# dingwentao/GPU-lossless-compression

Measured on AMD Instinct MI355X. Metric: encode+decode GB/s (input bytes) per GPU and whole-node; compression ratio parity, higher is better.
Workload: dtype u8; 1 GPU; configs[1]: 4 GiB/GPU Zipf(1.0) bytes (Philox4x32-10, key 0x5eed0002, counter = byte index / 4), 1 MiB blocks, cudppCompress BWT+MTF+Huffman encode; block_bytes=1048576, blocks_per_gpu=4096, batch_rows=2048, batch_rows_asked=2048, output_layout=compact, drain_between_steps=False, parallelism=blocks round-robin over 1 GPU(s), no data-path collective, blocks_left_by_bucket_sorter=0, blocks_left_by_sample_sorter=0

## Files before the change

### gpu-lossless-compression_amd/csrc/bwt_bucket.hip

```cpp
#include "glc_device.h"
#include "glc_internal.h"
#include "fs_words.h"

namespace glc {

constexpr int      FSS_NT    = 512;
constexpr int      FSS_ITEMS = FS_CAP / FSS_NT;
#ifndef GLC_FS_BIN_BITS
#define GLC_FS_BIN_BITS 12
#endif
constexpr uint32_t FS_BIN_BITS = GLC_FS_BIN_BITS, FS_BINS = 1u << FS_BIN_BITS;
#ifndef GLC_FSS_LOOK
#define GLC_FSS_LOOK 4
#endif
constexpr uint32_t FSS_LOOK = GLC_FSS_LOOK;
constexpr uint32_t FS_MAX_GROUP = 512;
constexpr uint32_t FS_START_MASK = 0x0FFFu, FS_BIG_BIN = 0x8000u;
static_assert(FS_FILLMAX <= FS_START_MASK, "a bin start and the end of the last bin fit below the big-bin flag");
constexpr uint32_t FSS_SENT = 2 * FSS_LOOK;

uint32_t fs_bucket_log2(uint32_t n)
{
    uint32_t l = 4;
    while (((uint64_t)FS_AVG << l) < n && l < FS_MAXNB_LOG2) l++;
    return l;
}

constexpr uint32_t FSH_SLICE = 32768;
constexpr uint32_t FSH_SLOTS = 2048, FS_DUP_FLAG = 48;

constexpr uint32_t FS_DONE = 8u;

__global__ __launch_bounds__(256) void k_fs_tables(const uint32_t *__restrict__ hist, uint32_t n,
                                                   uint2 *__restrict__ tab, const uint32_t *__restrict__ dup,
                                                   uint32_t *__restrict__ flag, const uint8_t *__restrict__ text, size_t stride,
                                                   uint8_t *__restrict__ bwt_out, size_t bwt_stride, int *__restrict__ d_index,
                                                   uint32_t *__restrict__ sa_out, size_t sa_stride, uint32_t step)
{
    __shared__ uint32_t s_tmp[5];
    const uint32_t b = blockIdx.x, tid = threadIdx.x;
    const uint32_t hraw = hist[(size_t)b * 256 + tid];
    const uint32_t h = hraw + (step > 1 ? 1u : 0u);
    uint32_t ns = 0;
    const uint32_t c = block_excl_add<256>(h, s_tmp, &ns);
    bool constant = __syncthreads_or((int)(hraw == ns - (step > 1 ? 256u : 0u))) != 0;
    if (constant && step > 1) {
        const uint8_t *T = text + (size_t)b * stride;
        const uint32_t sym = T[0];
        bool other = false;
        for (uint32_t i = tid; i < n && !other; i += 256) other = T[i] != sym;
        constant = __syncthreads_or((int)other) == 0;
    }
    if (tid == 0) {
        if (constant) flag[b] = FS_DONE;
        else if (dup[b] >= (FS_DUP_FLAG + step - 1) / step) flag[b] = 1u;
    }
    if (constant) {
        const uint32_t sym = text[(size_t)b * stride];
        const uint32_t v = sym * 0x01010101u;
        if (bwt_out) {
            uint8_t *O = bwt_out + (size_t)b * bwt_stride;
            const uint32_t head = min(n, (uint32_t)((16u - (uint32_t)(reinterpret_cast<uintptr_t>(O) & 15u)) & 15u));
            const uint32_t nvec = (n - head) / 16;
            for (uint32_t i = tid; i < head; i += 256) O[i] = (uint8_t)sym;
            for (uint32_t i = tid; i < nvec; i += 256) reinterpret_cast<uint4 *>(O + head)[i] = make_uint4(v, v, v, v);
            for (uint32_t i = head + nvec * 16 + tid; i < n; i += 256) O[i] = (uint8_t)sym;
        }
        if (sa_out) for (uint32_t i = tid; i < n; i += 256) sa_out[(size_t)b * sa_stride + i] = n - 1 - i;
        if (d_index && tid == 0) d_index[b] = (int)(n - 1);
        return;
    }
    const uint64_t C32 = ((uint64_t)c << 32) / ns, P32 = ((uint64_t)h << 32) / ns;
    tab[(size_t)b * 256 + tid] = make_uint2((uint32_t)(C32 > 0xFFFFFFFFull ? 0xFFFFFFFFull : C32),
                                            (uint32_t)(P32 > 0xFFFFFFFFull ? 0xFFFFFFFFull : P32));
}

#ifndef GLC_FSH_COPIES
#define GLC_FSH_COPIES 16
#endif
constexpr int FSH_COPIES = GLC_FSH_COPIES;
__global__ __launch_bounds__(256) void k_fs_hist(const uint8_t *__restrict__ text, size_t stride, uint32_t n,
                                                 uint32_t *__restrict__ hist, uint32_t *__restrict__ dup, uint32_t step)
{
    __shared__ uint32_t s_h[FSH_COPIES * 257];
    __shared__ uint32_t s_fp[FSH_SLOTS];
    __shared__ uint32_t s_dup;
    const uint32_t b = blockIdx.y, tid = threadIdx.x;
    const uint32_t lo = blockIdx.x * step * FSH_SLICE;
    if (lo >= n) return;
    const uint32_t hi = min(n, lo + FSH_SLICE);
    for (uint32_t i = tid; i < FSH_COPIES * 257; i += 256) s_h[i] = 0;
    for (uint32_t i = tid; i < FSH_SLOTS; i += 256) s_fp[i] = 0;
    if (tid == 0) s_dup = 0;
    __syncthreads();
    const uint8_t *T = text + (size_t)b * stride;
    uint32_t *H = s_h + (tid & (FSH_COPIES - 1)) * 257;
    uint32_t done = lo;
    if ((reinterpret_cast<uintptr_t>(T + lo) & 15) == 0) {
        const uint32_t nvec = (hi - lo) / 16;
        const uint4 *V = reinterpret_cast<const uint4 *>(T + lo);
        uint4 q[8];
#pragma unroll
        for (int r = 0; r < 8; r++) {
            const uint32_t i = r * 256 + tid;
            q[r] = i < nvec ? V[i] : make_uint4(0, 0, 0, 0);
        }
#pragma unroll
        for (int r = 0; r < 8; r += 4) {
            if (r * 256 + tid < nvec) {
                const uint32_t fp = (q[r].x * 0x9E3779B1u + (q[r].y & 0xFFFFu) * 0x85EBCA6Bu) | 1u;
                const uint32_t old = atomicCAS(&s_fp[(fp * 0xC2B2AE35u) >> 21], 0u, fp);
                if (old == fp) atomicAdd(&s_dup, 1u);
            }
        }
#pragma unroll
        for (int r = 0; r < 8; r++) {
            if (r * 256 + tid < nvec) {
                const uint32_t wd[4] = {q[r].x, q[r].y, q[r].z, q[r].w};
#pragma unroll
                for (int k = 0; k < 4; k++) {
                    atomicAdd(&H[wd[k] & 0xFF], 1u);
                    atomicAdd(&H[(wd[k] >> 8) & 0xFF], 1u);
                    atomicAdd(&H[(wd[k] >> 16) & 0xFF], 1u);
                    atomicAdd(&H[wd[k] >> 24], 1u);
                }
            }
        }
        done = lo + nvec * 16;
    }
    for (uint32_t i = done + tid; i < hi; i += 256) atomicAdd(&H[T[i]], 1u);
    __syncthreads();
    uint32_t c = 0;
#pragma unroll
    for (int k = 0; k < FSH_COPIES; k++) c += s_h[k * 257 + tid];
    if (c) atomicAdd(&hist[(size_t)b * 256 + tid], c);
    if (tid == 0 && s_dup) atomicAdd(&dup[b], s_dup);
}

#ifndef GLC_FSP2_T
#define GLC_FSP2_T 4
#endif
constexpr int FSP2_T = GLC_FSP2_T;
#ifndef GLC_FSP2_WAVES
#define GLC_FSP2_WAVES 5
#endif
#ifndef GLC_FSP2_NT
#define GLC_FSP2_NT 512
#endif
#ifndef GLC_FSP2_TILE
#define GLC_FSP2_TILE 4096
#endif
constexpr int FSP2_TILE = GLC_FSP2_TILE;
constexpr int FSP2_NT = GLC_FSP2_NT;

__device__ __forceinline__ void lds_only_barrier()
{
    asm volatile("s_waitcnt lgkmcnt(0)\n\ts_barrier" ::: "memory");
}

template <int NT>
__device__ __forceinline__ uint32_t bucket_excl_add_lds(uint32_t x, uint32_t *s_tmp)
{
    constexpr uint32_t NW = (NT < (int)FS_MAXNB ? NT : FS_MAXNB) / WAVE;
    const uint32_t w = __builtin_amdgcn_readfirstlane(threadIdx.x >> 6);
    const uint32_t inc = wave_incl_add(x);
    if ((threadIdx.x & 63) == 63 && w < NW) s_tmp[w] = inc;
    asm volatile("s_waitcnt lgkmcnt(0)\n\ts_barrier" ::: "memory");
    uint32_t base = 0;
#pragma unroll
    for (uint32_t i = 0; i < NW; i++)
        if (i < w) base += s_tmp[i];
    return base + inc - x;
}

template <int NT, int ITEMS, int WPE>
__global__ __launch_bounds__(NT) __attribute__((amdgpu_waves_per_eu(WPE, 8))) void k_fs_part2(const uint8_t *__restrict__ text, size_t stride, uint32_t n, uint32_t nbl,
                                                     const uint2 *__restrict__ tab, uint64_t *__restrict__ keys, size_t kstride,
                                                     uint32_t *__restrict__ fill, uint32_t *__restrict__ flag,
                                                     uint32_t *__restrict__ zero_bucket, uint32_t tiles_per_wg)
{
    constexpr uint32_t TILE = NT * ITEMS;
    __shared__ struct {
        uint32_t cnt[FS_MAXNB];
        uint16_t start[FS_MAXNB], gbase[FS_MAXNB];
        uint2 tab[256];
        uint32_t tmp[NT / 64 + 1];
        uint32_t flagged;
        uint64_t w[NT * ITEMS];
    } sh;
    uint32_t *s_cnt = sh.cnt, *s_tmp = sh.tmp;
    uint16_t *s_start = sh.start, *s_gbase = sh.gbase;
    uint2 *s_tab = sh.tab;
    uint64_t *s_w = sh.w;
    uint32_t &s_flagged = sh.flagged;
    uint8_t *s_txt = reinterpret_cast<uint8_t *>(s_w);
    uint32_t bx, by;
    xcd_order(bx, by);
    const uint32_t b = by, tid = threadIdx.x;
    const uint32_t ntiles = (n + TILE - 1) / TILE, tile0 = bx * tiles_per_wg;
    if (tile0 >= ntiles) return;
    const uint8_t *T = text + (size_t)b * stride;
    if (tid == 0) s_flagged = flag[b];
    if (tid < 256) s_tab[tid] = tab[(size_t)b * 256 + tid];
    constexpr int NSTG = ((TILE + 16) / 4 + NT - 1) / NT;
    uint32_t stg[NSTG] = {};
    auto inner = [&](uint32_t tile) { const uint32_t base = tile * TILE; return base > 0 && base + TILE + 16 <= n; };
    auto request = [&](uint32_t tile) {
        const uint8_t *D = T + (size_t)tile * TILE - 1;
#pragma unroll
        for (int r = 0; r < NSTG; r++) {
            const uint32_t q = r * NT + tid;
            const uint32_t qq = q < (TILE + 16) / 4 ? q : 0u;
            uint32_t v;
            __builtin_memcpy(&v, D + 4 * (size_t)qq, 4);
            stg[r] = v;
        }
    };
    const uint32_t tend = min(ntiles, tile0 + tiles_per_wg);
    bool have = false;
    if (inner(tile0)) { request(tile0); have = true; }
    uint64_t *K = keys + (size_t)b * kstride;
    static_assert(TILE <= (1u << 20), "a rank inside (tile, bucket) rides in the index field of the word until the scatter");
    constexpr uint32_t LOW = (uint32_t)FS_LOW_MASK;
    auto bucket_of = [&](uint32_t hi) { return __builtin_amdgcn_ubfe(hi, 32u - nbl, nbl); };
    auto tile_body = [&](auto edge_t, uint32_t base, bool next_inner) __attribute__((always_inline)) -> bool {
        constexpr bool EDGE = decltype(edge_t)::value;
        const uint32_t k0 = tid * ITEMS, gi0 = base + k0;
        constexpr int NBY = (ITEMS + FS_DEPTH + 3) / 4;
        uint32_t by4[NBY];
        if (ITEMS % 8 == 0) {
#pragma unroll
            for (int q = 0; q < NBY; q += 2) {
                const uint2 v = *reinterpret_cast<const uint2 *>(s_txt + k0 + 4 * q);
                by4[q] = v.x;
                if (q + 1 < NBY) by4[q + 1] = v.y;
            }
        } else {
#pragma unroll
            for (int q = 0; q < NBY; q++) by4[q] = *reinterpret_cast<const uint32_t *>(s_txt + k0 + 4 * q);
        }
#define FS_BYTE(j) ((by4[(j) >> 2] >> (8 * ((j) & 3))) & 0xFFu)
        uint2 e[ITEMS + FS_DEPTH - 1];
        auto entry = [&](int k) {
            const uint2 t = s_tab[FS_BYTE(1 + k)];
            if constexpr (EDGE) return gi0 + k >= n ? make_uint2(0u, 0u) : t;
            else return t;
        };
#pragma unroll
        for (int k = 0; k < FS_DEPTH - 1; k++) e[k] = entry(k);
        uint32_t xh[ITEMS], xl[ITEMS];
#pragma unroll
        for (int j = 0; j < ITEMS; j++) {
            e[j + FS_DEPTH - 1] = entry(j + FS_DEPTH - 1);
            uint32_t y = e[j + FS_DEPTH - 1].x;
#pragma unroll
            for (int d = FS_DEPTH - 2; d >= 1; d--) y = e[j + d].x + __umulhi(e[j + d].y, y);
            const uint64_t X = ((uint64_t)e[j].x << 32) + (uint64_t)e[j].y * y;
            const uint32_t hi = (uint32_t)(X >> 32), bk = bucket_of(hi);
            uint32_t r = 0;
            if (!EDGE || gi0 + j < n) r = atomicAdd(&s_cnt[bk], 1u);
            xh[j] = hi;
            xl[j] = ((uint32_t)X & ~LOW) | (r << 8);
            if (j == 0 && gi0 == 0) zero_bucket[b] = bk;
        }
        lds_only_barrier();
        uint32_t g = 0, c = 0;
        {
            c = tid < FS_MAXNB ? s_cnt[tid] : 0u;
            const uint32_t start = bucket_excl_add_lds<NT>(c, s_tmp);
            if (c) g = atomicAdd(&fill[(size_t)b * FS_MAXNB + tid], c);
            if (tid < FS_MAXNB) s_start[tid] = (uint16_t)start;
        }
        {
            const uint2 v = *reinterpret_cast<const uint2 *>(s_txt + k0);
            by4[0] = v.x;
            by4[1] = v.y;
#pragma unroll
            for (int j = 0; j < ITEMS; j++) xl[j] |= FS_BYTE(j);
        }
#undef FS_BYTE
        lds_only_barrier();
#pragma unroll
        for (int j = 0; j < ITEMS; j++) {
            asm volatile("" : "+v"(xh[j]), "+v"(xl[j]));
            if (!EDGE || gi0 + j < n) {
                const uint32_t lo = (xl[j] & ~(LOW ^ 0xFFu)) | ((gi0 + j) << 8);
                s_w[s_start[bucket_of(xh[j])] + ((xl[j] >> 8) & 0xFFFFFu)] = ((uint64_t)xh[j] << 32) | lo;
            }
        }
        if (c && g + c > FS_FILLMAX) { atomicOr(&flag[b], 1u); s_flagged = 1; }
        if (tid < FS_MAXNB) s_gbase[tid] = (uint16_t)(g < FS_CAP ? g : FS_CAP);
        if (next_inner) {
#pragma unroll
            for (int r = 0; r < NSTG; r++) asm volatile("" : "+v"(stg[r]));
        }
        lds_only_barrier();
        if constexpr (EDGE) {
            const uint32_t tile_n = min((uint32_t)TILE, n - base);
#pragma unroll
            for (int r = 0; r < ITEMS; r++) {
                const uint32_t p = r * NT + tid;
                if (p < tile_n) {
                    const uint64_t ww = s_w[p];
                    const uint32_t d = bucket_of((uint32_t)(ww >> 32));
                    const uint32_t off = (uint32_t)s_gbase[d] + (p - (uint32_t)s_start[d]);
                    if (off < FS_CAP) K[(size_t)d * FS_CAP + off] = ww;
                }
            }
        } else {
            if (__builtin_amdgcn_readfirstlane(s_flagged)) return false;
#pragma unroll
            for (int r = 0; r < ITEMS; r++) {
                const uint32_t p = r * NT + tid;
                const uint64_t ww = s_w[p];
                const uint32_t d = bucket_of((uint32_t)(ww >> 32));
                K[d * FS_CAP + (uint32_t)s_gbase[d] + (p - (uint32_t)s_start[d])] = ww;
            }
        }
        return true;
    };
#pragma clang loop unroll(disable)
    for (uint32_t tile = tile0; tile < tend; tile++) {
        const uint32_t base = tile * TILE;
        const bool edge = base + TILE + 16 > n;
        if (tid < FS_MAXNB) s_cnt[tid] = 0;
        if (have) {
#pragma unroll
            for (int r = 0; r < NSTG; r++) {
                const uint32_t q = r * NT + tid;
                if (q < (TILE + 16) / 4) reinterpret_cast<uint32_t *>(s_txt)[q] = stg[r];
            }
        } else {
            for (uint32_t k = tid; k < TILE + 16; k += NT) {
                const int64_t g = (int64_t)base - 1 + k;
                s_txt[k] = g < 0 ? T[n - 1] : (g < (int64_t)n ? T[g] : (uint8_t)0);
            }
        }
        lds_only_barrier();
        const bool next_inner = tile + 1 < tend && inner(tile + 1);
        if (next_inner) request(tile + 1);
        if (s_flagged) return;
        const bool go = edge ? tile_body(std::true_type{}, base, next_inner) : tile_body(std::false_type{}, base, next_inner);
        if (!go) return;
        have = next_inner;
        lds_only_barrier();
    }
}

__global__ __launch_bounds__(FS_MAXNB) void k_fs_scan(const uint32_t *__restrict__ fill, uint32_t *__restrict__ fbase,
                                                      uint32_t *__restrict__ flag, const uint32_t *__restrict__ list)
{
    __shared__ uint32_t s_tmp[FS_MAXNB / 64 + 1];
    const uint32_t b = list ? list[blockIdx.x] : blockIdx.x, tid = threadIdx.x;
    const uint32_t f = fill[(size_t)b * FS_MAXNB + tid];
    if (f > FS_FILLMAX) atomicOr(&flag[b], 1u);
    fbase[(size_t)b * FS_MAXNB + tid] = block_excl_add<FS_MAXNB>(f, s_tmp);
}

__global__ __launch_bounds__(FSS_NT) void k_fs_sort(uint32_t n, uint32_t nbl, const uint64_t *__restrict__ keys,
                                                    size_t kstride, const uint32_t *__restrict__ fill,
                                                    const uint32_t *__restrict__ fbase, uint32_t *__restrict__ flag,
                                                    uint8_t *__restrict__ bwt_out, size_t bwt_stride,
                                                    int *__restrict__ d_index, uint32_t *__restrict__ sa_out,
                                                    size_t sa_stride, uint4 *__restrict__ wl, uint32_t wl_cap,
                                                    uint32_t *__restrict__ wl_count)
{
    __shared__ uint64_t s_w[FS_FILLMAX + 4];
    __shared__ uint32_t s_cp[FS_BINS / 2 + 1];
    __shared__ uint32_t s_tmp[FSS_NT / 64 + 1];
    __shared__ uint32_t s_deep, s_wl;
    uint16_t *s16 = reinterpret_cast<uint16_t *>(s_cp);
    uint8_t *s_cb = reinterpret_cast<uint8_t *>(s_cp);
    uint32_t gx, gy;
    xcd_order(gx, gy);
    const uint32_t b = gy, bk = gx, tid = threadIdx.x;
    if (tid == 0) { s_deep = flag[b]; s_wl = 0; }
    for (uint32_t i = tid; i < FS_BINS / 2; i += FSS_NT) s_cp[i] = 0;
    const uint32_t c = fill[(size_t)b * FS_MAXNB + bk];
    const uint32_t R0 = fbase[(size_t)b * FS_MAXNB + bk];
    const uint64_t *K = keys + (size_t)b * kstride + (size_t)bk * FS_CAP;
    uint64_t w[FSS_ITEMS];
#pragma unroll
    for (int r = 0; r < FSS_ITEMS; r++) {
        const uint32_t i = r * FSS_NT + tid;
        w[r] = ~0ull;
        if (r * FSS_NT < c && c <= FS_FILLMAX && i < c) w[r] = K[i];
    }
    if (tid < 4 && c <= FS_FILLMAX) s_w[c + tid] = ~0ull;
    __syncthreads();
    if (s_deep || c == 0) return;
    const uint32_t bshift = 64 - nbl - FS_BIN_BITS;
    uint32_t rk[FSS_ITEMS];
#pragma unroll
    for (int r = 0; r < FSS_ITEMS; r++) {
        rk[r] = 0;
        if (r * FSS_NT >= c) continue;
        const uint32_t i = r * FSS_NT + tid;
        const uint32_t bin = (uint32_t)(w[r] >> bshift) & (FS_BINS - 1), sh = 16 * (bin & 1);
        if (i < c) rk[r] = (atomicAdd(&s_cp[bin >> 1], 1u << sh) >> sh) & 0xFFFFu;
    }
    __syncthreads();
    {
        constexpr int PW = FS_BINS / 2 / FSS_NT;
        uint32_t v[PW], sum = 0;
#pragma unroll
        for (int k = 0; k < PW; k++) { v[k] = s_cp[tid * PW + k]; sum += (v[k] & 0xFFFFu) + (v[k] >> 16); }
        uint32_t run = block_excl_add<FSS_NT>(sum, s_tmp);
#pragma unroll
        for (int k = 0; k < PW; k++) {
            const uint32_t lo = run, hi = run + (v[k] & 0xFFFFu);
            s_cp[tid * PW + k] = lo | (hi << 16);
            run = hi + (v[k] >> 16);
        }
        if (tid == FSS_NT - 1) s_cp[FS_BINS / 2] = c;
    }
    __syncthreads();
#pragma unroll
    for (int r = 0; r < FSS_ITEMS; r++) {
        if (r * FSS_NT >= c) continue;
        const uint32_t i = r * FSS_NT + tid;
        if (i < c) s_w[s16[(uint32_t)(w[r] >> bshift) & (FS_BINS - 1)] + rk[r]] = w[r];
    }
    __syncthreads();
    uint32_t *SAo = sa_out ? sa_out + (size_t)b * sa_stride + R0 : nullptr;
    uint32_t pos[FSS_ITEMS], grp[FSS_ITEMS];
#pragma unroll
    for (int r = 0; r < FSS_ITEMS; r++) {
        const uint32_t p = r * FSS_NT + tid;
        pos[r] = 0xFFFFFFFFu; grp[r] = 0;
        if (r * FSS_NT >= c) continue;
        if (p < c) {
            const uint64_t wv = s_w[p];
            w[r] = wv;
            const uint32_t key = (uint32_t)(wv >> 28);
            const uint32_t bin = (uint32_t)(wv >> bshift) & (FS_BINS - 1);
            const uint32_t gs = s16[bin], ge = s16[bin + 1];
            if (ge - gs > FS_MAX_GROUP) { s_deep = 1; }
            else {
                uint32_t less = 0, eqt = 0;
                const uint2 *B = reinterpret_cast<const uint2 *>(s_w) + gs;
#pragma unroll
                for (uint32_t t = 0; t < 4; t++) {
                    const uint2 wq = B[t];
                    const uint32_t kq = __builtin_amdgcn_alignbit(wq.y, wq.x, 28);
                    less += kq < key ? 1u : 0u;
                    eqt += kq == key ? 1u : 0u;
                }
                if (ge - gs > 4) {
#pragma clang loop unroll(disable)
                    for (uint32_t q = gs + 4; q < ge; q++) {
                        const uint2 wq = reinterpret_cast<const uint2 *>(s_w)[q];
                        const uint32_t kq = __builtin_amdgcn_alignbit(wq.y, wq.x, 28);
                        less += kq < key; eqt += kq == key;
                    }
                }
                const uint32_t idx = (uint32_t)(wv >> 8) & 0xFFFFFu;
                uint32_t at = gs + less;
                if (eqt > 1) {
                    uint32_t eqb = 0; eqt = 0;
#pragma clang loop unroll(disable)
                    for (uint32_t q = gs; q < ge; q++) {
                        const uint2 wq = reinterpret_cast<const uint2 *>(s_w)[q];
                        const bool e = __builtin_amdgcn_alignbit(wq.y, wq.x, 28) == key;
                        eqt += e; eqb += e & (q < p);
                    }
                    if (eqt > 1) { grp[r] = (at << 16) | eqt; at += eqb; }
                }
                pos[r] = at;
                if (!grp[r]) {
                    if (SAo) SAo[at] = idx;
                    if (idx == 0 && d_index) d_index[b] = (int)(R0 + at);
                }
            }
        }
    }
    __syncthreads();
    if (s_deep) { if (tid == 0) atomicOr(&flag[b], 2u); return; }
    uint8_t *O = bwt_out ? bwt_out + (size_t)b * bwt_stride + R0 : nullptr;
    const uint32_t shift = (uint32_t)(reinterpret_cast<uintptr_t>(O) & 3u);
    bool any = false;
#pragma unroll
    for (int r = 0; r < FSS_ITEMS; r++) {
        if (pos[r] != 0xFFFFFFFFu) s_cb[shift + pos[r]] = (uint8_t)w[r];
        if (grp[r]) {
            any = true;
            const uint32_t gp = grp[r] >> 16, gs = grp[r] & 0xFFFFu;
            if (pos[r] == gp) reinterpret_cast<uint32_t *>(s_w)[2 * gp + 1] = atomicAdd(&s_wl, gs);
        }
    }
    if (__syncthreads_or((int)any)) {
        if (tid == 0) {
            const uint32_t tot = s_wl;
            uint32_t base = atomicAdd(&wl_count[b], tot);
            if (base + tot > wl_cap) { atomicOr(&flag[b], 4u); base = 0xFFFFFFFFu; }
            s_deep = base;
        }
        __syncthreads();
        const uint32_t base = s_deep;
        uint4 *WL = wl + (size_t)b * wl_cap;
        if (base != 0xFFFFFFFFu) {
#pragma unroll
            for (int r = 0; r < FSS_ITEMS; r++) {
                if (grp[r]) {
                    const uint32_t gp = grp[r] >> 16, gs = grp[r] & 0xFFFFu, slot0 = base + reinterpret_cast<const uint32_t *>(s_w)[2 * gp + 1];
                    WL[slot0 + (pos[r] - gp)] = make_uint4((uint32_t)(w[r] & FS_LOW_MASK), R0 + gp, slot0, gs);
                }
            }
        }
    }
    if (O) {
        const uint32_t end = shift + c;
        for (uint32_t q = tid; 4 * q < end; q += FSS_NT) {
            const uint32_t v = s_cp[q];
            if (4 * q >= shift && 4 * q + 4 <= end) *reinterpret_cast<uint32_t *>(O - shift + 4 * q) = v;
            else {
#pragma unroll
                for (uint32_t k = 0; k < 4; k++)
                    if (4 * q + k >= shift && 4 * q + k < end) O[4 * q + k - shift] = (uint8_t)(v >> (8 * k));
            }
        }
    }
}

__global__ __launch_bounds__(FSS_NT) __attribute__((amdgpu_waves_per_eu(8, 8))) void k_fs_sort_bwt(uint32_t nbl, const uint64_t *__restrict__ keys, size_t kstride,
                                                        const uint32_t *__restrict__ fill, const uint32_t *__restrict__ fbase,
                                                        uint32_t *__restrict__ flag, uint8_t *__restrict__ bwt_out,
                                                        size_t bwt_stride, int *__restrict__ d_index, uint4 *__restrict__ wl,
                                                        uint32_t wl_cap, uint32_t *__restrict__ wl_count,
                                                        const uint32_t *__restrict__ zero_bucket)
{
    __shared__ uint64_t s_w[FS_FILLMAX + FSS_SENT];
    __shared__ uint32_t s_cp[FS_BINS / 2 + 1];
    __shared__ uint32_t s_tmp[FSS_NT / 64 + 1];
    __shared__ uint32_t s_deep, s_wl;
    uint16_t *s16 = reinterpret_cast<uint16_t *>(s_cp);
    uint8_t *s_cb = reinterpret_cast<uint8_t *>(s_cp);
    uint32_t gx, gy;
    xcd_order(gx, gy);
    const uint32_t b = gy, bk = gx, tid = threadIdx.x;
    if (scalar_load_u32(flag + b) & (1u | FS_DONE)) return;
    if (tid == 0) { s_deep = flag[b]; s_wl = 0; }
    for (uint32_t i = tid; i < FS_BINS / 2; i += FSS_NT) s_cp[i] = 0;
    const uint64_t *K = keys + (size_t)b * kstride + (size_t)bk * FS_CAP;
    constexpr int FSS_SPEC = 3;
    uint64_t ws[FSS_SPEC + 1];
#pragma unroll
    for (int r = 1; r <= FSS_SPEC; r++) ws[r] = K[(r - 1) * FSS_NT + tid];
    const uint32_t c = fill[(size_t)b * FS_MAXNB + bk];
    const uint32_t R0 = fbase[(size_t)b * FS_MAXNB + bk];
    const bool zb = zero_bucket[b] == bk;
    const uint32_t cc = c <= FS_FILLMAX ? c : 0u;
    const uint32_t full = cc / FSS_NT, part = cc % FSS_NT;
    const bool v0 = tid < part;
    const uint32_t i0 = full * FSS_NT + tid;
    const uint32_t bshift = 64 - nbl - FS_BIN_BITS;
    const uint32_t hshift = bshift - 32, kshift = bshift - 28;
    uint8_t *O = bwt_out + (size_t)b * bwt_stride + R0;
    const uint32_t shift = (uint32_t)(reinterpret_cast<uintptr_t>(O) & 3u);

    auto bin_starts = [&]() __attribute__((always_inline)) {
        constexpr int PW = FS_BINS / 2 / FSS_NT;
        uint32_t v[PW], sum = 0;
#pragma unroll
        for (int k = 0; k < PW; k++) { v[k] = s_cp[tid * PW + k]; sum += (v[k] & 0xFFFFu) + (v[k] >> 16); }
        uint32_t run = block_excl_add<FSS_NT>(sum, s_tmp);
#pragma unroll
        for (int k = 0; k < PW; k++) {
            const uint32_t lo = run, hi = run + (v[k] & 0xFFFFu);
            s_cp[tid * PW + k] = lo | (hi << 16);
            run = hi + (v[k] >> 16);
        }
        if (tid == FSS_NT - 1) s_cp[FS_BINS / 2] = c;
    };
    auto sorted_word = [](uint64_t wv) -> uint64_t {
        const uint32_t lo = (uint32_t)wv, hi = (uint32_t)(wv >> 32);
        return ((uint64_t)__builtin_amdgcn_alignbit(hi, lo, 28) << 32) | lo;
    };
    auto rank_rare = [&](uint32_t key, uint32_t p, uint32_t gs, uint32_t ge, uint32_t &at, uint32_t &grp) __attribute__((always_inline)) {
        if (ge - gs > FS_MAX_GROUP) { s_deep = 1; at = 0xFFFFFFFFu; }
        else {
            uint32_t ls = 0, eq = 0, eqb = 0;
#pragma clang loop unroll(disable)
            for (uint32_t q = gs; q < ge; q++) {
                const uint32_t kq = reinterpret_cast<const uint32_t *>(s_w)[2 * q + 1];
                ls += kq < key; eq += kq == key; eqb += (kq == key) & (q < p);
            }
            at = gs + ls;
            if (eq > 1) { grp = (at << 16) | eq; at += eqb; }
        }
    };
    auto rank_rare2 = [&](uint32_t key, uint32_t p, uint32_t gs, const uint32_t *k1, uint32_t &at, uint32_t &grp) __attribute__((always_inline)) {
        const uint32_t *B = reinterpret_cast<const uint32_t *>(s_w) + 2 * (gs + FSS_LOOK) + 1;
        uint32_t k2[FSS_LOOK];
#pragma unroll
        for (uint32_t t = 0; t < FSS_LOOK; t++) k2[t] = B[2 * t];
        const uint32_t ge = s16[((key >> kshift) & (FS_BINS - 1)) + 1] & FS_START_MASK;
        if ((ge - gs > 2 * FSS_LOOK) | (key == 0xFFFFFFFFu)) rank_rare(key, p, gs, ge, at, grp);
        else {
            uint32_t ls = 0, em = 0;
#pragma unroll
            for (uint32_t t = 0; t < 2 * FSS_LOOK; t++) {
                const uint32_t kq = t < FSS_LOOK ? k1[t < FSS_LOOK ? t : 0] : k2[t < FSS_LOOK ? 0 : t - FSS_LOOK];
                ls += kq < key ? 1u : 0u;
                em |= kq == key ? 1u << t : 0u;
            }
            const uint32_t eq = __builtin_popcount(em);
            at = gs + ls;
            if (eq > 1) { grp = (at << 16) | eq; at += __builtin_popcount(em & ((1u << (p - gs)) - 1u)); }
        }
    };
    auto wl_reserve = [&](uint32_t pos, uint32_t grp) __attribute__((always_inline)) {
        const uint32_t gp = grp >> 16, gs = grp & 0xFFFFu;
        if (pos == gp) reinterpret_cast<uint32_t *>(s_w)[2 * gp + 1] = atomicAdd(&s_wl, gs);
    };
    auto wl_base = [&]() __attribute__((always_inline)) -> uint32_t {
        __syncthreads();
        const uint32_t tot = s_wl;
        if (tot == 0) return 0xFFFFFFFFu;
        if (tid == 0) {
            uint32_t base = atomicAdd(&wl_count[b], tot);
            if (base + tot > wl_cap) { atomicOr(&flag[b], 4u); base = 0xFFFFFFFFu; }
            s_deep = base;
        }
        __syncthreads();
        return s_deep;
    };
    auto wl_entry = [&](uint32_t base, uint64_t wv, uint32_t pos, uint32_t grp) __attribute__((always_inline)) {
        uint4 *WL = wl + (size_t)b * wl_cap;
        const uint32_t gp = grp >> 16, gs = grp & 0xFFFFu, slot0 = base + reinterpret_cast<const uint32_t *>(s_w)[2 * gp + 1];
        WL[slot0 + (pos - gp)] = make_uint4((uint32_t)(wv & FS_LOW_MASK), R0 + gp, slot0, gs);
    };

    auto rounds = [&](auto full_t) __attribute__((always_inline)) -> bool {
        constexpr int FULL = decltype(full_t)::value, NS = FULL + 1;
        static_assert(FULL >= FSS_SPEC && NS <= FSS_ITEMS, "the requested rounds are all full ones");
        uint64_t w[NS];
        w[0] = ~0ull;
        if (v0) w[0] = K[i0];
#pragma unroll
        for (int r = 1; r <= FULL; r++) w[r] = r <= FSS_SPEC ? ws[r <= FSS_SPEC ? r : 0] : K[(r - 1) * FSS_NT + tid];
        if (tid < FSS_SENT) s_w[cc + tid] = ~0ull;
        __syncthreads();
        if (s_deep) return false;
        uint32_t bin[NS], rk[NS];
#pragma unroll
        for (int r = 0; r < NS; r++) bin[r] = ((uint32_t)(w[r] >> 32) >> hshift) & (FS_BINS - 1);
        rk[0] = 0;
        if (v0) rk[0] = atomicAdd(&s_cp[bin[0] >> 1], 1u << (16 * (bin[0] & 1)));
#pragma unroll
        for (int r = 1; r < NS; r++) rk[r] = atomicAdd(&s_cp[bin[r] >> 1], 1u << (16 * (bin[r] & 1)));
#pragma unroll
        for (int r = 0; r < NS; r++) rk[r] = (rk[r] >> (16 * (bin[r] & 1))) & 0xFFFFu;
        __syncthreads();
        bin_starts();
        __syncthreads();
        {
            uint32_t st[NS];
            st[0] = 0;
            if (v0) st[0] = s16[bin[0]];
#pragma unroll
            for (int r = 1; r < NS; r++) st[r] = s16[bin[r]];
            bool late = false;
#pragma unroll
            for (int r = 0; r < NS; r++) late |= rk[r] >= FSS_LOOK;
            if (late) {
#pragma unroll
                for (int r = 0; r < NS; r++)
                    if (rk[r] >= FSS_LOOK) atomicOr(&s_cp[bin[r] >> 1], FS_BIG_BIN << (16 * (bin[r] & 1)));
            }
#pragma unroll
            for (int r = 0; r < NS; r++) rk[r] += st[r] & FS_START_MASK;
            if (v0) s_w[rk[0]] = sorted_word(w[0]);
        }
#pragma unroll
        for (int r = 1; r < NS; r++) s_w[rk[r]] = sorted_word(w[r]);
        __syncthreads();
        uint32_t pos[NS], grp[NS], gs[NS];
        bool big[NS];
        if (v0) w[0] = s_w[i0];
#pragma unroll
        for (int r = 1; r < NS; r++) w[r] = s_w[(r - 1) * FSS_NT + tid];
        gs[0] = 0;
        if (v0) gs[0] = s16[((uint32_t)(w[0] >> 32) >> kshift) & (FS_BINS - 1)];
#pragma unroll
        for (int r = 1; r < NS; r++) gs[r] = s16[((uint32_t)(w[r] >> 32) >> kshift) & (FS_BINS - 1)];
#pragma unroll
        for (int r = 0; r < NS; r++) { big[r] = gs[r] > FS_START_MASK; gs[r] &= FS_START_MASK; }
        uint32_t kq[NS][FSS_LOOK];
        if (v0) {
            const uint32_t *B = reinterpret_cast<const uint32_t *>(s_w) + 2 * gs[0] + 1;
#pragma unroll
            for (uint32_t t = 0; t < FSS_LOOK; t++) kq[0][t] = B[2 * t];
        }
#pragma unroll
        for (int r = 1; r < NS; r++) {
            const uint32_t *B = reinterpret_cast<const uint32_t *>(s_w) + 2 * gs[r] + 1;
#pragma unroll
            for (uint32_t t = 0; t < FSS_LOOK; t++) kq[r][t] = B[2 * t];
        }
        bool rare[NS], rare_any = false;
#pragma unroll
        for (int r = 0; r < NS; r++) {
            const uint32_t key = (uint32_t)(w[r] >> 32);
            uint32_t less = 0, eqt = 0;
#pragma unroll
            for (uint32_t t = 0; t < FSS_LOOK; t++) {
                less += kq[r][t] < key ? 1u : 0u;
                eqt += kq[r][t] == key ? 1u : 0u;
            }
            pos[r] = gs[r] + less; grp[r] = 0;
            rare[r] = (big[r] | (eqt > 1)) & (r > 0 || v0);
            rare_any |= rare[r];
        }
        if (__builtin_amdgcn_ballot_w64(rare_any) != 0) {
#pragma unroll
            for (int r = 0; r < NS; r++)
                if (rare[r]) rank_rare2((uint32_t)(w[r] >> 32), r ? (r - 1) * FSS_NT + tid : i0, gs[r], kq[r], pos[r], grp[r]);
        }
        if (zb) {
            asm volatile("" ::: "memory");
#pragma unroll
            for (int r = 0; r < NS; r++)
                if ((r > 0 || v0) && pos[r] != 0xFFFFFFFFu && ((uint32_t)w[r] & 0x0FFFFF00u) == 0 && !grp[r]) d_index[b] = (int)(R0 + pos[r]);
        }
        __syncthreads();
        if (s_deep) { if (tid == 0) atomicOr(&flag[b], 2u); return false; }
        if (v0) s_cb[shift + pos[0]] = (uint8_t)w[0];
#pragma unroll
        for (int r = 1; r < NS; r++) s_cb[shift + pos[r]] = (uint8_t)w[r];
        uint32_t tied = 0;
#pragma unroll
        for (int r = 0; r < NS; r++) tied |= grp[r];
        if (tied) {
#pragma unroll
            for (int r = 0; r < NS; r++)
                if (grp[r]) wl_reserve(pos[r], grp[r]);
        }
        const uint32_t base = wl_base();
        if (base != 0xFFFFFFFFu && tied) {
#pragma unroll
            for (int r = 0; r < NS; r++)
                if (grp[r]) wl_entry(base, w[r], pos[r], grp[r]);
        }
        return true;
    };

    auto guarded = [&]() __attribute__((always_inline)) -> bool {
        uint64_t w[FSS_ITEMS];
#pragma unroll
        for (int r = 0; r < FSS_ITEMS; r++) w[r] = r >= 1 && r <= FSS_SPEC ? ws[r >= 1 && r <= FSS_SPEC ? r : 0] : ~0ull;
        if (v0) w[0] = K[i0];
#pragma unroll
        for (int r = FSS_SPEC + 1; r < FSS_ITEMS; r++)
            if ((uint32_t)r <= full) w[r] = K[(r - 1) * FSS_NT + tid];
        if (tid < FSS_SENT && cc) s_w[cc + tid] = ~0ull;
        __syncthreads();
        if (s_deep || cc == 0) return false;
        uint32_t rk[FSS_ITEMS];
#pragma unroll
        for (int r = 0; r < FSS_ITEMS; r++) rk[r] = 0;
        {
            auto count = [&](int r) {
                const uint32_t bin = ((uint32_t)(w[r] >> 32) >> hshift) & (FS_BINS - 1), sh = 16 * (bin & 1);
                rk[r] = (atomicAdd(&s_cp[bin >> 1], 1u << sh) >> sh) & 0xFFFFu;
            };
            if (v0) count(0);
#pragma unroll
            for (int r = 1; r < FSS_ITEMS; r++)
                if ((uint32_t)r <= full) count(r);
        }
        __syncthreads();
        bin_starts();
        __syncthreads();
        {
            auto scatter = [&](int r) {
                const uint32_t bin = ((uint32_t)(w[r] >> 32) >> hshift) & (FS_BINS - 1);
                const uint32_t st = s16[bin];
                if (rk[r] >= FSS_LOOK) atomicOr(&s_cp[bin >> 1], FS_BIG_BIN << (16 * (bin & 1)));
                s_w[(st & FS_START_MASK) + rk[r]] = sorted_word(w[r]);
            };
            if (v0) scatter(0);
#pragma unroll
            for (int r = 1; r < FSS_ITEMS; r++)
                if ((uint32_t)r <= full) scatter(r);
        }
        __syncthreads();
        uint32_t pos[FSS_ITEMS], grp[FSS_ITEMS];
#pragma unroll
        for (int r = 0; r < FSS_ITEMS; r++) { pos[r] = 0xFFFFFFFFu; grp[r] = 0; }
        {
            auto rank = [&](int r, uint32_t p) {
                const uint64_t wv = s_w[p];
                w[r] = wv;
                const uint32_t key = (uint32_t)(wv >> 32);
                const uint32_t bin = (key >> kshift) & (FS_BINS - 1);
                const uint32_t gf = s16[bin], gs = gf & FS_START_MASK;
                uint32_t less = 0, eqt = 0, kq[FSS_LOOK];
                const uint32_t *B = reinterpret_cast<const uint32_t *>(s_w) + 2 * gs + 1;
#pragma unroll
                for (uint32_t t = 0; t < FSS_LOOK; t++) {
                    kq[t] = B[2 * t];
                    less += kq[t] < key ? 1u : 0u;
                    eqt += kq[t] == key ? 1u : 0u;
                }
                uint32_t at = gs + less;
                const bool rare = (gf > FS_START_MASK) | (eqt > 1);
                if (__builtin_amdgcn_ballot_w64(rare) != 0) {
                    if (rare) rank_rare2(key, p, gs, kq, at, grp[r]);
                }
                pos[r] = at;
            };
            if (v0) rank(0, i0);
#pragma unroll
            for (int r = 1; r < FSS_ITEMS; r++)
                if ((uint32_t)r <= full) rank(r, (r - 1) * FSS_NT + tid);
            if (zb) {
                asm volatile("" ::: "memory");
#pragma unroll
                for (int r = 0; r < FSS_ITEMS; r++)
                    if (pos[r] != 0xFFFFFFFFu && ((uint32_t)w[r] & 0x0FFFFF00u) == 0 && !grp[r]) d_index[b] = (int)(R0 + pos[r]);
            }
        }
        __syncthreads();
        if (s_deep) { if (tid == 0) atomicOr(&flag[b], 2u); return false; }
#pragma unroll
        for (int r = 0; r < FSS_ITEMS; r++) {
            if (pos[r] != 0xFFFFFFFFu) s_cb[shift + pos[r]] = (uint8_t)w[r];
            if (grp[r]) wl_reserve(pos[r], grp[r]);
        }
        const uint32_t base = wl_base();
        if (base != 0xFFFFFFFFu) {
#pragma unroll
            for (int r = 0; r < FSS_ITEMS; r++)
                if (grp[r]) wl_entry(base, w[r], pos[r], grp[r]);
        }
        return true;
    };

    const bool go = full == 3 ? rounds(std::integral_constant<int, 3>{}) : full == 4 ? rounds(std::integral_constant<int, 4>{}) : guarded();
    if (!go) return;
    {
        const uint32_t end = shift + c;
        for (uint32_t q = tid; 4 * q < end; q += FSS_NT) {
            const uint32_t v = s_cp[q];
            if (4 * q >= shift && 4 * q + 4 <= end) *reinterpret_cast<uint32_t *>(O - shift + 4 * q) = v;
            else {
#pragma unroll
                for (uint32_t k = 0; k < 4; k++)
                    if (4 * q + k >= shift && 4 * q + k < end) O[4 * q + k - shift] = (uint8_t)(v >> (8 * k));
            }
        }
    }
}

#ifndef GLC_FST_W
#define GLC_FST_W 4
#endif
constexpr int FST_W = GLC_FST_W;
__global__ __launch_bounds__(256) void k_fs_ties(const uint8_t *__restrict__ text, size_t stride, uint32_t n,
                                                 const uint4 *__restrict__ wl, uint32_t wl_cap,
                                                 const uint32_t *__restrict__ wl_count, uint32_t *__restrict__ flag,
                                                 uint8_t *__restrict__ bwt_out, size_t bwt_stride,
                                                 int *__restrict__ d_index, uint32_t *__restrict__ sa_out, size_t sa_stride)
{
    uint32_t gx, gy;
    xcd_order(gx, gy);
    const uint32_t b = gy;
    const uint32_t total = wl_count[b];
    if (total == 0 || total > wl_cap || flag[b]) return;
    const uint4 *WL = wl + (size_t)b * wl_cap;
    const uint8_t *T = text + (size_t)b * stride;
    for (uint32_t e = gx * 256 + threadIdx.x; e < total; e += gridDim.x * 256) {
        const uint4 me = WL[e];
        const uint32_t gs = me.w, idx = me.x >> 8;
        uint32_t rank = 0;
        bool deep = false;
        const bool fast_me = idx + 12 <= n;
        const uint64_t mine = fast_me ? fs_load_be64(T + idx) : 0ull;
        for (uint32_t f0 = me.z; f0 < me.z + gs && !deep; f0 += FST_W) {
            uint32_t oi[FST_W];
            uint64_t ov[FST_W];
#pragma unroll
            for (int k = 0; k < FST_W; k++) oi[k] = f0 + k < me.z + gs ? WL[f0 + k].x >> 8 : idx;
#pragma unroll
            for (int k = 0; k < FST_W; k++) ov[k] = (oi[k] != idx && fast_me && oi[k] + 12 <= n) ? fs_load_be64(T + oi[k]) : mine;
#pragma unroll
            for (int k = 0; k < FST_W; k++) {
                if (oi[k] == idx) continue;
                if (fast_me && oi[k] + 12 <= n && ov[k] != mine) rank += ov[k] < mine ? 1u : 0u;
                else rank += fs_suffix_less(T, n, oi[k], idx, &deep) ? 1u : 0u;
            }
        }
        if (deep) { atomicOr(&flag[b], 2u); continue; }
        const uint32_t row = me.y + rank;
        if (bwt_out) bwt_out[(size_t)b * bwt_stride + row] = (uint8_t)me.x;
        if (sa_out) sa_out[(size_t)b * sa_stride + row] = idx;
        if (idx == 0 && d_index) d_index[b] = (int)row;
    }
}

__global__ void k_fs_finish(const uint32_t *__restrict__ flag, uint32_t n, uint32_t nblk, uint32_t *__restrict__ lcnt,
                            uint32_t *__restrict__ nflag, uint32_t *__restrict__ redo, uint32_t *__restrict__ keep,
                            uint32_t *__restrict__ list, uint32_t *__restrict__ h_nflag, const uint32_t *__restrict__ dup,
                            uint32_t dup_flag)
{
    __shared__ uint32_t s_last;
    const uint32_t b = blockIdx.x * blockDim.x + threadIdx.x;
    if (b < nblk) {
        const uint32_t f = (flag[b] && flag[b] != FS_DONE) ? n : 0u;
        lcnt[b] = f;
        redo[b] = f;
        keep[b] = f ? 0u : 1u;
        if (f) list[atomicAdd(nflag, 1u)] = b;
        if (flag[b] != FS_DONE && dup[b] < dup_flag) atomicAdd(nflag + 4, 1u);
    }
    __threadfence();
    __syncthreads();
    if (threadIdx.x == 0) s_last = atomicAdd(&nflag[3], 1u) == gridDim.x - 1 ? 1u : 0u;
    __syncthreads();
    if (s_last && threadIdx.x == 0) {
        __threadfence();
        reinterpret_cast<volatile uint32_t *>(h_nflag)[1] = atomicAdd(nflag + 4, 0u);
        *reinterpret_cast<volatile uint32_t *>(h_nflag) = atomicAdd(nflag, 0u);
        __threadfence_system();
    }
}

__global__ __launch_bounds__(256) void k_fs_clear(uint32_t nblk, uint32_t *__restrict__ hist, uint32_t *__restrict__ fill,
                                                  uint32_t *__restrict__ flag, uint32_t flag_value, uint32_t *__restrict__ wlcnt,
                                                  uint32_t *__restrict__ dup, uint32_t *__restrict__ nflag)
{
    const uint32_t nh = nblk * 256u, nf = nblk * FS_MAXNB, total = nh + nf + 3u * nblk + 8u;
    for (uint32_t i = blockIdx.x * 256u + threadIdx.x; i < total; i += gridDim.x * 256u) {
        if (i < nh) hist[i] = 0;
        else if (i < nh + nf) fill[i - nh] = 0;
        else {
            const uint32_t j = i - nh - nf;
            if (j < nblk) flag[j] = flag_value;
            else if (j < 2 * nblk) wlcnt[j - nblk] = 0;
            else if (j < 3 * nblk) dup[j - 2 * nblk] = 0;
            else nflag[j - 3 * nblk] = 0;
        }
    }
}

hipError_t fs_scan(hipStream_t st, uint32_t nlisted, const uint32_t *fill, uint32_t *fbase, uint32_t *flag, const uint32_t *list)
{
    hipLaunchKernelGGL(k_fs_scan, dim3(nlisted), dim3(FS_MAXNB), 0, st, fill, fbase, flag, list);
    return hipGetLastError();
}

hipError_t fs_build(const SortCall &c, SaScratch &s)
{
    const hipStream_t st = c.st;
    const uint8_t *const text = c.text;
    const size_t text_stride = c.text_stride, bwt_stride = c.bwt_stride;
    const uint32_t n = c.n, nblk = c.nblk;
    uint8_t *const bwt_out = c.bwt_out;
    int *const d_index = c.d_index;
    uint32_t *const sa_out = c.sa_out(s);
    const uint32_t nbl = fs_bucket_log2(n), nb = 1u << nbl;
    {
        const uint32_t words = nblk * (256u + FS_MAXNB + 3u) + 8u, g = (words + 1023) / 1024;
        hipLaunchKernelGGL(k_fs_clear, dim3(g < 2048 ? g : 2048), dim3(256), 0, st, nblk, s.fs_hist, s.fs_fill, s.fs_flag,
                           s.skip_tier1 ? 1u : 0u, s.fs_wlcnt, s.fs_dup, s.fs_nflag);
    }
    uint32_t *h_nflag = s.h_max_cnt + HW_FLAGGED;
    const double units = (double)n * nblk;
    const uint32_t nslices = (n + FSH_SLICE - 1) / FSH_SLICE;
    const uint32_t hstep = nslices >= 16 ? 4u : 1u;
    {
        ProfScope ps(s.prof, PROF_FS_HIST, st, units);
        hipLaunchKernelGGL(k_fs_hist, dim3((nslices + hstep - 1) / hstep, nblk), dim3(256), 0, st, text, text_stride, n,
                           s.fs_hist, s.fs_dup, hstep);
    }
    hipLaunchKernelGGL(k_fs_tables, dim3(nblk), dim3(256), 0, st, s.fs_hist, n, s.fs_tab, s.fs_dup, s.fs_flag, text, text_stride,
                       bwt_out, bwt_stride, d_index, sa_out, (size_t)s.nmax, hstep);
    if (s.skip_tier1) {
        hipLaunchKernelGGL(k_fs_finish, dim3((nblk + 255) / 256), dim3(256), 0, st, s.fs_flag, n, nblk, s.fs_lcnt, s.fs_nflag,
                           s.fs_redo[s.parity & 1], s.fs_keep[s.parity & 1], s.ss_list, h_nflag, s.fs_dup, (FS_DUP_FLAG + hstep - 1) / hstep);
        return hipGetLastError();
    }
    {
        ProfScope ps(s.prof, PROF_FS_PART, st, units);
        if (nblk >= 16) {
#ifndef GLC_FSP2_BT
#define GLC_FSP2_BT 8192
#endif
            constexpr int BT = GLC_FSP2_BT, BN = 1024;
            const uint32_t tiles = (n + BT - 1) / BT, per = 16;
            hipLaunchKernelGGL((k_fs_part2<BN, BT / BN, 4>), dim3((tiles + per - 1) / per, nblk), dim3(BN), 0, st, text, text_stride, n, nbl,
                               s.fs_tab, s.keyA, s.fs_kstride, s.fs_fill, s.fs_flag, s.fs_zero, per);
        } else {
            const uint32_t tiles = (n + FSP2_TILE - 1) / FSP2_TILE;
            const uint32_t per = nblk >= 4 ? FSP2_T : 1u;
            hipLaunchKernelGGL((k_fs_part2<FSP2_NT, FSP2_TILE / FSP2_NT, GLC_FSP2_WAVES>), dim3((tiles + per - 1) / per, nblk), dim3(FSP2_NT), 0, st,
                               text, text_stride, n, nbl, s.fs_tab, s.keyA, s.fs_kstride, s.fs_fill, s.fs_flag, s.fs_zero, per);
        }
    }
    hipLaunchKernelGGL(k_fs_scan, dim3(nblk), dim3(FS_MAXNB), 0, st, s.fs_fill, s.fs_base, s.fs_flag, (const uint32_t *)nullptr);
    {
        ProfScope ps(s.prof, PROF_FS_SORT, st, units);
        if (sa_out || !bwt_out || !d_index)
            hipLaunchKernelGGL(k_fs_sort, dim3(nb, nblk), dim3(FSS_NT), 0, st, n, nbl, s.keyA, s.fs_kstride, s.fs_fill, s.fs_base, s.fs_flag,
                               bwt_out, bwt_stride, d_index, sa_out, (size_t)s.nmax, s.fs_wl, s.fs_wl_cap, s.fs_wlcnt);
        else
            hipLaunchKernelGGL(k_fs_sort_bwt, dim3(nb, nblk), dim3(FSS_NT), 0, st, nbl, s.keyA, s.fs_kstride, s.fs_fill, s.fs_base, s.fs_flag,
                               bwt_out, bwt_stride, d_index, s.fs_wl, s.fs_wl_cap, s.fs_wlcnt, s.fs_zero);
    }
    hipLaunchKernelGGL(k_fs_ties, dim3(24, nblk), dim3(256), 0, st, text, text_stride, n, s.fs_wl, s.fs_wl_cap, s.fs_wlcnt,
                       s.fs_flag, bwt_out, bwt_stride, d_index, sa_out, (size_t)s.nmax);
    hipLaunchKernelGGL(k_fs_finish, dim3((nblk + 255) / 256), dim3(256), 0, st, s.fs_flag, n, nblk, s.fs_lcnt, s.fs_nflag,
                       s.fs_redo[s.parity & 1], s.fs_keep[s.parity & 1], s.ss_list, h_nflag, s.fs_dup, (FS_DUP_FLAG + hstep - 1) / hstep);
    return hipGetLastError();
}

}
```

Before: 122.7 GB/s.

## Feed inner tiles' text bytes straight from registers, skipping LDS staging

For interior tiles, each thread now loads its own 16 bytes of text with one vector load into registers and uses them directly for the code computation. This replaces staging the tile into LDS and reading it back, which also removes a barrier per tile. The loop is restructured so edge tiles keep the LDS path while runs of interior tiles prefetch the next tile's registers. s_cnt is cleared inside the body instead of at the top of each tile. It relies on ITEMS==8 and FS_DEPTH==8 (static_assert), and the reworked barrier ordering between edge and inner tiles adds correctness risk.

```diff
diff --git a/gpu-lossless-compression_amd/csrc/bwt_bucket.hip b/gpu-lossless-compression_amd/csrc/bwt_bucket.hip
--- a/gpu-lossless-compression_amd/csrc/bwt_bucket.hip
+++ b/gpu-lossless-compression_amd/csrc/bwt_bucket.hip
@@ -202,42 +202,36 @@
     const uint8_t *T = text + (size_t)b * stride;
     if (tid == 0) s_flagged = flag[b];
     if (tid < 256) s_tab[tid] = tab[(size_t)b * 256 + tid];
-    constexpr int NSTG = ((TILE + 16) / 4 + NT - 1) / NT;
-    uint32_t stg[NSTG] = {};
+    if (tid < FS_MAXNB) s_cnt[tid] = 0;
+    static_assert(ITEMS == 8 && FS_DEPTH == 8, "a thread's codes and BWT bytes come from the 16 bytes of one load");
+    constexpr int NBY = (ITEMS + FS_DEPTH + 3) / 4;
+    uint32_t nxt[NBY] = {};
     auto inner = [&](uint32_t tile) { const uint32_t base = tile * TILE; return base > 0 && base + TILE + 16 <= n; };
     auto request = [&](uint32_t tile) {
-        const uint8_t *D = T + (size_t)tile * TILE - 1;
-#pragma unroll
-        for (int r = 0; r < NSTG; r++) {
-            const uint32_t q = r * NT + tid;
-            const uint32_t qq = q < (TILE + 16) / 4 ? q : 0u;
-            uint32_t v;
-            __builtin_memcpy(&v, D + 4 * (size_t)qq, 4);
-            stg[r] = v;
-        }
+        uint4 v;
+        __builtin_memcpy(&v, T + (size_t)tile * TILE - 1 + ITEMS * tid, 16);
+        nxt[0] = v.x; nxt[1] = v.y; nxt[2] = v.z; nxt[3] = v.w;
     };
     const uint32_t tend = min(ntiles, tile0 + tiles_per_wg);
-    bool have = false;
-    if (inner(tile0)) { request(tile0); have = true; }
+    if (inner(tile0)) request(tile0);
     uint64_t *K = keys + (size_t)b * kstride;
     static_assert(TILE <= (1u << 20), "a rank inside (tile, bucket) rides in the index field of the word until the scatter");
     constexpr uint32_t LOW = (uint32_t)FS_LOW_MASK;
     auto bucket_of = [&](uint32_t hi) { return __builtin_amdgcn_ubfe(hi, 32u - nbl, nbl); };
-    auto tile_body = [&](auto edge_t, uint32_t base, bool next_inner) __attribute__((always_inline)) -> bool {
+    auto tile_body = [&](auto edge_t, uint32_t base, const uint32_t (&txt)[NBY]) __attribute__((always_inline)) -> bool {
         constexpr bool EDGE = decltype(edge_t)::value;
         const uint32_t k0 = tid * ITEMS, gi0 = base + k0;
-        constexpr int NBY = (ITEMS + FS_DEPTH + 3) / 4;
         uint32_t by4[NBY];
-        if (ITEMS % 8 == 0) {
-#pragma unroll
-            for (int q = 0; q < NBY; q += 2) {
+#pragma unroll
+        for (int q = 0; q < NBY; q += 2) {
+            if constexpr (EDGE) {
                 const uint2 v = *reinterpret_cast<const uint2 *>(s_txt + k0 + 4 * q);
                 by4[q] = v.x;
-                if (q + 1 < NBY) by4[q + 1] = v.y;
-            }
-        } else {
-#pragma unroll
-            for (int q = 0; q < NBY; q++) by4[q] = *reinterpret_cast<const uint32_t *>(s_txt + k0 + 4 * q);
+                by4[q + 1] = v.y;
+            } else {
+                by4[q] = txt[q];
+                by4[q + 1] = txt[q + 1];
+            }
         }
 #define FS_BYTE(j) ((by4[(j) >> 2] >> (8 * ((j) & 3))) & 0xFFu)
         uint2 e[ITEMS + FS_DEPTH - 1];
@@ -267,14 +261,17 @@
         uint32_t g = 0, c = 0;
         {
             c = tid < FS_MAXNB ? s_cnt[tid] : 0u;
+            if (tid < FS_MAXNB) s_cnt[tid] = 0;
             const uint32_t start = bucket_excl_add_lds<NT>(c, s_tmp);
             if (c) g = atomicAdd(&fill[(size_t)b * FS_MAXNB + tid], c);
             if (tid < FS_MAXNB) s_start[tid] = (uint16_t)start;
         }
         {
-            const uint2 v = *reinterpret_cast<const uint2 *>(s_txt + k0);
-            by4[0] = v.x;
-            by4[1] = v.y;
+            if constexpr (EDGE) {
+                const uint2 v = *reinterpret_cast<const uint2 *>(s_txt + k0);
+                by4[0] = v.x;
+                by4[1] = v.y;
+            }
 #pragma unroll
             for (int j = 0; j < ITEMS; j++) xl[j] |= FS_BYTE(j);
         }
@@ -290,10 +287,8 @@
         }
         if (c && g + c > FS_FILLMAX) { atomicOr(&flag[b], 1u); s_flagged = 1; }
         if (tid < FS_MAXNB) s_gbase[tid] = (uint16_t)(g < FS_CAP ? g : FS_CAP);
-        if (next_inner) {
-#pragma unroll
-            for (int r = 0; r < NSTG; r++) asm volatile("" : "+v"(stg[r]));
-        }
+#pragma unroll
+        for (int r = 0; r < NBY; r++) asm volatile("" : "+v"(nxt[r]));
         lds_only_barrier();
         if constexpr (EDGE) {
             const uint32_t tile_n = min((uint32_t)TILE, n - base);
@@ -319,31 +314,38 @@
         }
         return true;
     };
+    lds_only_barrier();
+#pragma unroll
+    for (int r = 0; r < NBY; r++) asm volatile("" : "+v"(nxt[r]));
+    uint32_t tile = tile0;
 #pragma clang loop unroll(disable)
-    for (uint32_t tile = tile0; tile < tend; tile++) {
-        const uint32_t base = tile * TILE;
-        const bool edge = base + TILE + 16 > n;
-        if (tid < FS_MAXNB) s_cnt[tid] = 0;
-        if (have) {
-#pragma unroll
-            for (int r = 0; r < NSTG; r++) {
-                const uint32_t q = r * NT + tid;
-                if (q < (TILE + 16) / 4) reinterpret_cast<uint32_t *>(s_txt)[q] = stg[r];
-            }
-        } else {
+    while (tile < tend) {
+        if (__builtin_amdgcn_readfirstlane(s_flagged)) return;
+        if (!inner(tile)) {
+            const uint32_t base = tile * TILE;
+            if (tile != tile0) lds_only_barrier();
             for (uint32_t k = tid; k < TILE + 16; k += NT) {
                 const int64_t g = (int64_t)base - 1 + k;
                 s_txt[k] = g < 0 ? T[n - 1] : (g < (int64_t)n ? T[g] : (uint8_t)0);
             }
-        }
-        lds_only_barrier();
-        const bool next_inner = tile + 1 < tend && inner(tile + 1);
-        if (next_inner) request(tile + 1);
-        if (s_flagged) return;
-        const bool go = edge ? tile_body(std::true_type{}, base, next_inner) : tile_body(std::false_type{}, base, next_inner);
-        if (!go) return;
-        have = next_inner;
-        lds_only_barrier();
+            lds_only_barrier();
+            if (tile + 1 < tend && inner(tile + 1)) request(tile + 1);
+            tile_body(std::true_type{}, base, nxt);
+            tile++;
+            continue;
+        }
+        bool next_inner;
+#pragma clang loop unroll(disable)
+        do {
+            uint32_t txt[NBY];
+#pragma unroll
+            for (int q = 0; q < NBY; q++) txt[q] = nxt[q];
+            next_inner = tile + 1 < tend && inner(tile + 1);
+            if (next_inner) request(tile + 1);
+            if (!tile_body(std::false_type{}, tile * TILE, txt)) return;
+            lds_only_barrier();
+            tile++;
+        } while (next_inner);
     }
 }
 
```

Result: no change. 121.9 GB/s (-0.6%).

## Split inner-tile key build into load/compute/atomic phases and separate edge loop

Applied to the files above, without the earlier changes.

For interior tiles the bucket-scatter kernel now loads every lookup-table entry first, then computes all codes and LDS atomics, then reads the bucket starts before the scatter stores. Scheduling barriers mark the phase boundaries so LDS loads can be batched and their latency overlapped. The tile loop is restructured so edge tiles take a separate path and interior tiles run in a tight inner loop with the prefetch. This raises register pressure (all entries live at once) and may reduce occupancy.

```diff
diff --git a/gpu-lossless-compression_amd/csrc/bwt_bucket.hip b/gpu-lossless-compression_amd/csrc/bwt_bucket.hip
--- a/gpu-lossless-compression_amd/csrc/bwt_bucket.hip
+++ b/gpu-lossless-compression_amd/csrc/bwt_bucket.hip
@@ -152,6 +152,9 @@
 #endif
 constexpr int FSP2_TILE = GLC_FSP2_TILE;
 constexpr int FSP2_NT = GLC_FSP2_NT;
+#ifndef GLC_FSP2_PHASES
+#define GLC_FSP2_PHASES 1
+#endif
 
 __device__ __forceinline__ void lds_only_barrier()
 {
@@ -217,14 +220,13 @@
         }
     };
     const uint32_t tend = min(ntiles, tile0 + tiles_per_wg);
-    bool have = false;
-    if (inner(tile0)) { request(tile0); have = true; }
     uint64_t *K = keys + (size_t)b * kstride;
     static_assert(TILE <= (1u << 20), "a rank inside (tile, bucket) rides in the index field of the word until the scatter");
     constexpr uint32_t LOW = (uint32_t)FS_LOW_MASK;
     auto bucket_of = [&](uint32_t hi) { return __builtin_amdgcn_ubfe(hi, 32u - nbl, nbl); };
     auto tile_body = [&](auto edge_t, uint32_t base, bool next_inner) __attribute__((always_inline)) -> bool {
         constexpr bool EDGE = decltype(edge_t)::value;
+        constexpr bool PHASES = !EDGE && WPE <= 4 && GLC_FSP2_PHASES;
         const uint32_t k0 = tid * ITEMS, gi0 = base + k0;
         constexpr int NBY = (ITEMS + FS_DEPTH + 3) / 4;
         uint32_t by4[NBY];
@@ -246,22 +248,43 @@
             if constexpr (EDGE) return gi0 + k >= n ? make_uint2(0u, 0u) : t;
             else return t;
         };
-#pragma unroll
-        for (int k = 0; k < FS_DEPTH - 1; k++) e[k] = entry(k);
+        auto code = [&](int j) {
+            uint32_t y = e[j + FS_DEPTH - 1].x;
+#pragma unroll
+            for (int d = FS_DEPTH - 2; d >= 1; d--) y = e[j + d].x + __umulhi(e[j + d].y, y);
+            return ((uint64_t)e[j].x << 32) + (uint64_t)e[j].y * y;
+        };
         uint32_t xh[ITEMS], xl[ITEMS];
-#pragma unroll
-        for (int j = 0; j < ITEMS; j++) {
-            e[j + FS_DEPTH - 1] = entry(j + FS_DEPTH - 1);
-            uint32_t y = e[j + FS_DEPTH - 1].x;
-#pragma unroll
-            for (int d = FS_DEPTH - 2; d >= 1; d--) y = e[j + d].x + __umulhi(e[j + d].y, y);
-            const uint64_t X = ((uint64_t)e[j].x << 32) + (uint64_t)e[j].y * y;
-            const uint32_t hi = (uint32_t)(X >> 32), bk = bucket_of(hi);
-            uint32_t r = 0;
-            if (!EDGE || gi0 + j < n) r = atomicAdd(&s_cnt[bk], 1u);
-            xh[j] = hi;
-            xl[j] = ((uint32_t)X & ~LOW) | (r << 8);
-            if (j == 0 && gi0 == 0) zero_bucket[b] = bk;
+        if constexpr (PHASES) {
+#pragma unroll
+            for (int k = 0; k < ITEMS + FS_DEPTH - 1; k++) e[k] = entry(k);
+            __builtin_amdgcn_sched_barrier(0);
+            uint32_t rk[ITEMS];
+#pragma unroll
+            for (int j = 0; j < ITEMS; j++) {
+                const uint64_t X = code(j);
+                xh[j] = (uint32_t)(X >> 32);
+                xl[j] = (uint32_t)X & ~LOW;
+                rk[j] = atomicAdd(&s_cnt[bucket_of(xh[j])], 1u);
+            }
+            __builtin_amdgcn_sched_barrier(0);
+#pragma unroll
+            for (int j = 0; j < ITEMS; j++) xl[j] |= rk[j] << 8;
+        } else {
+#pragma unroll
+            for (int k = 0; k < FS_DEPTH - 1; k++) e[k] = entry(k);
+#pragma unroll
+            for (int j = 0; j < ITEMS; j++) {
+                e[j + FS_DEPTH - 1] = entry(j + FS_DEPTH - 1);
+                if constexpr (EDGE) if (j > 0) asm volatile("" : "+v"(xl[j - 1]));
+                const uint64_t X = code(j);
+                const uint32_t hi = (uint32_t)(X >> 32), bk = bucket_of(hi);
+                uint32_t r = 0;
+                if (!EDGE || gi0 + j < n) r = atomicAdd(&s_cnt[bk], 1u);
+                xh[j] = hi;
+                xl[j] = ((uint32_t)X & ~LOW) | (r << 8);
+                if constexpr (EDGE) if (j == 0 && gi0 == 0) zero_bucket[b] = bk;
+            }
         }
         lds_only_barrier();
         uint32_t g = 0, c = 0;
@@ -280,12 +303,23 @@
         }
 #undef FS_BYTE
         lds_only_barrier();
-#pragma unroll
-        for (int j = 0; j < ITEMS; j++) {
-            asm volatile("" : "+v"(xh[j]), "+v"(xl[j]));
-            if (!EDGE || gi0 + j < n) {
+        if constexpr (PHASES) {
+            uint32_t at[ITEMS];
+#pragma unroll
+            for (int j = 0; j < ITEMS; j++) at[j] = s_start[bucket_of(xh[j])];
+#pragma unroll
+            for (int j = 0; j < ITEMS; j++) {
                 const uint32_t lo = (xl[j] & ~(LOW ^ 0xFFu)) | ((gi0 + j) << 8);
-                s_w[s_start[bucket_of(xh[j])] + ((xl[j] >> 8) & 0xFFFFFu)] = ((uint64_t)xh[j] << 32) | lo;
+                s_w[at[j] + ((xl[j] >> 8) & 0xFFFFFu)] = ((uint64_t)xh[j] << 32) | lo;
+            }
+        } else {
+#pragma unroll
+            for (int j = 0; j < ITEMS; j++) {
+                asm volatile("" : "+v"(xh[j]), "+v"(xl[j]));
+                if (!EDGE || gi0 + j < n) {
+                    const uint32_t lo = (xl[j] & ~(LOW ^ 0xFFu)) | ((gi0 + j) << 8);
+                    s_w[s_start[bucket_of(xh[j])] + ((xl[j] >> 8) & 0xFFFFFu)] = ((uint64_t)xh[j] << 32) | lo;
+                }
             }
         }
         if (c && g + c > FS_FILLMAX) { atomicOr(&flag[b], 1u); s_flagged = 1; }
@@ -319,31 +353,45 @@
         }
         return true;
     };
+    uint32_t tile = tile0;
+    if (inner(tile)) request(tile);
 #pragma clang loop unroll(disable)
-    for (uint32_t tile = tile0; tile < tend; tile++) {
-        const uint32_t base = tile * TILE;
-        const bool edge = base + TILE + 16 > n;
-        if (tid < FS_MAXNB) s_cnt[tid] = 0;
-        if (have) {
+    while (tile < tend) {
+        if (!inner(tile)) {
+            const uint32_t base = tile * TILE;
+            if (tid < FS_MAXNB) s_cnt[tid] = 0;
+            for (uint32_t k = tid; k < TILE + 16; k += NT) {
+                const int64_t g = (int64_t)base - 1 + k;
+                s_txt[k] = g < 0 ? T[n - 1] : (g < (int64_t)n ? T[g] : (uint8_t)0);
+            }
+            lds_only_barrier();
+            if (s_flagged) return;
+            const bool next_inner = tile + 1 < tend && inner(tile + 1);
+            if (next_inner) request(tile + 1);
+            tile_body(std::true_type{}, base, next_inner);
+            lds_only_barrier();
+            tile++;
+            continue;
+        }
+#pragma unroll
+        for (int r = 0; r < NSTG; r++) asm volatile("" : "+v"(stg[r]));
+#pragma clang loop unroll(disable)
+        for (;;) {
+            if (tid < FS_MAXNB) s_cnt[tid] = 0;
 #pragma unroll
             for (int r = 0; r < NSTG; r++) {
                 const uint32_t q = r * NT + tid;
                 if (q < (TILE + 16) / 4) reinterpret_cast<uint32_t *>(s_txt)[q] = stg[r];
             }
-        } else {
-            for (uint32_t k = tid; k < TILE + 16; k += NT) {
-                const int64_t g = (int64_t)base - 1 + k;
-                s_txt[k] = g < 0 ? T[n - 1] : (g < (int64_t)n ? T[g] : (uint8_t)0);
-            }
-        }
-        lds_only_barrier();
-        const bool next_inner = tile + 1 < tend && inner(tile + 1);
-        if (next_inner) request(tile + 1);
-        if (s_flagged) return;
-        const bool go = edge ? tile_body(std::true_type{}, base, next_inner) : tile_body(std::false_type{}, base, next_inner);
-        if (!go) return;
-        have = next_inner;
-        lds_only_barrier();
+            lds_only_barrier();
+            if (s_flagged) return;
+            const bool more = tile + 1 < tend && inner(tile + 1);
+            if (more) request(tile + 1);
+            if (!tile_body(std::false_type{}, tile * TILE, more)) return;
+            lds_only_barrier();
+            tile++;
+            if (!more) break;
+        }
     }
 }
 
```

Result: faster. 121.7 GB/s before, 123.2 GB/s after, median of 6 (+1.2%).
